# godhj93/bayesian-torch

Measured on AMD Instinct MI355X. Metric: MC-samples/sec (forward+KL), Bayesian-ResNet18 CIFAR batch=128, higher is better.
Workload: dtype f32 (bf16x3 split operands, 6 product terms, f32 accumulate); 1 GPU; cfg3: Bayesian-ResNet18 via dnn_to_bnn (Conv2dReparameterization), CIFAR 3x32x32, batch=128; samples_per_launch=32, batch=128, rng=on-chip philox, parallelism=mc1, output_stage=bn+relu+residual (+ the stem max-pool) folded into the conv kernels, launch=hip graph replay

## Files before the change

### bayesian_torch_amd/_lib.py

```python
import ctypes as C
import os
import threading

import torch

_HERE = os.path.dirname(os.path.abspath(__file__))
LIB_PATH = os.environ.get("BT_LIB_PATH") or os.path.join(_HERE, "libbtorch_hip.so")
WORKSPACE_BYTES = 65536
KL_MAX_SEGMENTS = 64
PACK_MAX_SEGMENTS = 64
KL_RHO_IS_SIGMA = 1
KL_PRIOR_LAPLACE = 2
PRIOR_NORMAL, PRIOR_LAPLACE = 0, 1

_f32p = C.POINTER(C.c_float)
_vp = C.c_void_p


class bt_rng(C.Structure):
    _fields_ = [("seed", C.c_uint64), ("call_base_dev", _vp), ("call", C.c_uint32), ("layer_id", C.c_uint32),
                ("sample0", C.c_uint32), ("reserved", C.c_uint32)]


class bt_params(C.Structure):
# ... 59 lines not shown
    "bt_mc_epilogue": (C.c_int, [C.c_int32, C.c_int32, C.c_int32, _vp, _vp, _vp]),
}
EXPORTS = tuple(_PROTOS)


def lib():
    global _lib
    if _lib is None:
        with _lock:
            if _lib is None:
                if not os.path.exists(LIB_PATH):
                    raise RuntimeError(
                        f"{LIB_PATH} is missing: the HIP extension is the only implementation of this path "
                        "(no CPU/ATen fallback). Build it with `python -c 'import __graft_entry__ as g; g.build()'` "
                        "or `make -C bayesian_torch_amd/csrc`.")
                handle = C.CDLL(LIB_PATH)
                for name, (res, args) in _PROTOS.items():
                    fn = getattr(handle, name)
                    fn.restype, fn.argtypes = res, args
                _lib = handle
    return _lib


LAUNCH_INFO_FIELDS = ("workgroups", "m_tiles", "n_tiles", "S", "t_NI", "t_R", "t_Wt", "pixel_major", "row_tiles", "kl_slices", "groups", "n_bt", "n_rt", "n_ct", "fused_kl")


def last_launch_info():
    v = (C.c_int64 * 16)()
    check(lib().bt_last_launch_info(v, 16))
    return dict(zip(LAUNCH_INFO_FIELDS, (int(x) for x in v)))


ERR_UNSUPPORTED = -2


def check(rc):
    if rc != 0:
        raise RuntimeError(f"libbtorch_hip error {rc}: {lib().bt_last_error_string().decode()}")


def ptr(t):
    return None if t is None else t.data_ptr()


def dev_f32(t, what):
    if t is None:
        return None
# ... 63 lines not shown
```

### bayesian_torch_amd/csrc/bt_fused_api.hip

```cpp
#include <string.h>

#include "bt_fused_fwd.h"

namespace bt {
int launch_reparam(bool linear, const FwdArgs& a, FwdArgs& ran, hipStream_t stream);
int launch_reparam_inj(bool linear, const FwdArgs& a, FwdArgs& ran, hipStream_t stream);
int launch_flipout(bool linear, const FwdArgs& a, FwdArgs& ran, hipStream_t stream);
int launch_flipout_inj(bool linear, const FwdArgs& a, FwdArgs& ran, hipStream_t stream);

static unsigned long long* g_dbg = nullptr;
static thread_local long long g_launch_info[16] = {};
static inline bool al16(const void* p) { return (((uintptr_t)p) & 15u) == 0; }

static int run(bool flip, bool linear, const bt_conv2d_geom& g, int S, const float* x, int64_t x_sample_stride, const bt_params* p,
               const bt_draws* d, const bt_epilogue* ep, float* out, float* kl_out, void* ws, size_t ws_bytes, bt_stream_t stream, const char* who) {
  char msg[256];
  auto bad = [&](const char* what) {
    snprintf(msg, sizeof(msg), "%s: %s", who, what);
    return set_error(BT_ERR_BAD_ARG, msg);
  };
  if (!x || !p || !d || !out) return bad("null argument");
  if (!p->mu_w || !p->rho_w) return bad("mu_w / rho_w are required");
  if ((p->mu_b == nullptr) != (p->rho_b == nullptr)) return bad("mu_b and rho_b must both be given or both be NULL");
  if (S <= 0) return bad("S must be >= 1");
// ... 58 lines not shown
  a.seed_lo = (uint32_t)d->rng.seed, a.seed_hi = (uint32_t)(d->rng.seed >> 32);
  if (ep) a.ep_scale = ep->scale, a.ep_shift = ep->shift, a.ep_res = ep->residual, a.ep_res_stride = ep->residual_sample_stride, a.ep_relu = ep->relu;
  if (ep && ep->pool != BT_POOL_NONE) {
    if (ep->pool != BT_POOL_MAX_3x3_S2_P1) return bad("unknown epilogue pool mode");
    if (linear) return bad("the fused max-pool belongs to the conv2d entry points");
    if (ep->residual) return bad("the fused max-pool takes no residual");
    a.ep_pool = 1, a.ep_Hp = (Ho - 1) / 2 + 1, a.ep_Wp = (Wo - 1) / 2 + 1;
    a.out_elems = (long long)g.B * g.Co * a.ep_Hp * a.ep_Wp;
  }
  a.out_vec4 = (!linear && !a.pixel_major && a.HoWo > 1 && (a.Wo & 3) == 0 && al16(out) && (!a.ep_res || (al16(a.ep_res) && (a.ep_res_stride & 3) == 0)) &&
                (!d->sign_out || al16(d->sign_out))) ? 1 : 0;
  a.dbg = g_dbg;
  a.call = d->rng.call, a.call_base = d->rng.call_base_dev, a.layer_id = d->rng.layer_id, a.sample0 = d->rng.sample0;
  const bool inj = d->eps_w != nullptr;
  const bool all_inj = inj && (!p->mu_b || d->eps_b) && (!flip || (d->sign_in && d->sign_out));
  const bool none_inj = !d->eps_w && !d->eps_b && !d->sign_in && !d->sign_out;
  if (!all_inj && !none_inj) return bad("inject all draws of the layer (eps_w, eps_b when biased, both sign tensors for Flipout) or none");
  if (inj && a.ep_pool) return set_error(BT_ERR_UNSUPPORTED, "fused max-pool: not available with injected draws");
  int rc;
  FwdArgs r;
  if (inj) rc = flip ? launch_flipout_inj(linear, a, r, (hipStream_t)stream) : launch_reparam_inj(linear, a, r, (hipStream_t)stream);
  else rc = flip ? launch_flipout(linear, a, r, (hipStream_t)stream) : launch_reparam(linear, a, r, (hipStream_t)stream);
  if (rc == BT_OK) {
    const long long v[16] = {r.total_blocks, r.m_tiles, r.n_tiles, r.S, r.t_NI, r.t_R, r.t_Wt, r.pixel_major, r.row_taps, r.kl_slices, r.G, r.n_bt, r.n_rt, r.n_ct, r.do_kl, 0};
    for (int i = 0; i < 16; ++i) g_launch_info[i] = v[i];
  }
  if (rc == BT_OK && kl_after) {
    const float* mu[2] = {p->mu_w, p->mu_b};
    const float* rho[2] = {p->rho_w, p->rho_b};
    const float* pm[2] = {p->prior_mu_w, p->prior_mu_b};
    const float* ps[2] = {p->prior_sigma_w, p->prior_sigma_b};
    const int64_t n[2] = {a.w_elems, (int64_t)g.Co};
    const int32_t lay[2] = {0, 0};
    rc = bt_kl_normal(p->mu_b ? 2 : 1, mu, rho, pm, ps, n, lay, BT_KL_PRIOR_LAPLACE, kl_out, ws, ws_bytes, stream);
  }
  return rc;
}

static bt_conv2d_geom linear_geom(int B, int In, int Out) {
  bt_conv2d_geom g;
  g.B = B, g.Ci = In, g.H = 1, g.W = 1, g.Co = Out, g.kh = 1, g.kw = 1;
  g.sh = g.sw = 1, g.ph = g.pw = 0, g.dh = g.dw = 1, g.groups = 1;
  return g;
}
}

extern "C" int bt_reparam_linear_fwd(int32_t B, int32_t In, int32_t Out, int32_t S, const float* x, int64_t x_sample_stride,
// ... 35 lines not shown
```

### bayesian_torch_amd/csrc/bt_fused_fwd.h

```cpp
#pragma once
#include <type_traits>

#include "bt_api_internal.h"

namespace bt {

typedef float f32x16 __attribute__((ext_vector_type(16)));

constexpr int kBK = 36;
constexpr int kMaxTaps = 128;
#ifndef BT_STAMPS
#define BT_STAMPS 0
#endif
constexpr bool kStamps = BT_STAMPS != 0;
constexpr int kThreads = 512;
constexpr int kProducers = 256;

struct FwdArgs {
  const float *x, *mu_w, *rho_w, *mu_b, *rho_b, *pmu_w, *psig_w, *pmu_b, *psig_b;
  const float *mu_pk, *sig_pk;
  const float *eps_w, *eps_b, *sign_in, *sign_out;
  float* out;
  float* kl_out;
  double* slots;
  unsigned* counter;
  long long x_sample_stride, x_elems, out_elems, w_elems;
  int B, Ci, H, W, Co, KH, KW, SH, SW, PH, PW, DH, DW, G;
  int Ho, Wo, HoWo, M, K, Cig, Cog, S, T, HW;
  int n_tiles, m_tiles, total_blocks;
  int t_NI, t_R, t_Wt, n_bt, n_rt, n_ct;
  int patch_ok;
  int x_cvec;
  int x_rows;
  int pixel_major, mt_per_pixel;
  int w_vec, x_vec;
  int do_kl, kl_slices;
  uint32_t seed_lo, seed_hi, call, layer_id, sample0;
  const uint32_t* call_base;
  const float *ep_scale, *ep_shift, *ep_res;
  long long ep_res_stride;
  int ep_relu;
  int ep_pool, ep_Hp, ep_Wp;
  int out_vec4;
  int bn32;
  unsigned long long* dbg;
  uint32_t inv_m_tiles, inv_S, inv_n_tiles, inv_n_bt, inv_n_ct, inv_rw, inv_wt, inv_kw;
  int x_flat;
  int row_taps;
  float* sk_scratch;
  unsigned* sk_tickets;
  long long sk_scratch_bytes;
  int sk_nsl, sk_ks, sk_cpt;
  int sk_kh0, sk_nh, sk_kw0, sk_nw;
  int d_tap;
  int spw, n_sg;
  uint32_t inv_n_sg;
};

inline bool set_grid(FwdArgs& a, long long total) {
  if (total <= 0 || total > 0x7FFFFFFFll) return false;
  a.total_blocks = (int)total;
  a.kl_slices = total < 256 ? (int)total : 256;
  return true;
}

inline bool packed_ok(const FwdArgs& a) {
  return a.mu_pk && !((((uintptr_t)a.mu_pk | (uintptr_t)a.sig_pk) & 15u)) && a.w_elems < (1ll << 29) && a.x_elems < (1ll << 29);
}

__device__ __forceinline__ int xcd_remap(int orig, int n) {
// ... 740 lines not shown
```

### bayesian_torch_amd/csrc/bt_fused_split.h

```cpp
#pragma once
#include "bt_fused_fwd.h"

namespace bt {

typedef short bf16x8 __attribute__((ext_vector_type(8)));

constexpr int kSplitSteps = 5;

template <int BM, bool FLIP = false>
constexpr int split_xpo() {
  return FLIP ? 302 : 1025;
}
template <int BN, int NP, bool FLIP = false>
constexpr int split_w_bytes() { return (FLIP ? 2 : 1) * kSplitSteps * 2 * NP * BN * 16; }
template <int BM, int NP, bool FLIP = false>
constexpr int split_x_bytes() { return split_xpo<BM, FLIP>() * (NP + (FLIP ? 1 : 0)) * 16; }
constexpr int kSplitMiscBytes = kMaxTaps * 16 + 96 + 32 + 64;
template <int BN, int BM, int NP, bool FLIP = false>
constexpr int split_lds_bytes() { return 2 * (split_w_bytes<BN, NP, FLIP>() + split_x_bytes<BM, NP, FLIP>()) + kSplitMiscBytes; }

__device__ __forceinline__ void split_pieces(float v, uint32_t& h, uint32_t& m, uint32_t& l) {
  h = __float_as_uint(v) & 0xFFFF0000u;
  const float r = __fsub_rn(v, __uint_as_float(h));
  m = __float_as_uint(r) & 0xFFFF0000u;
  l = __float_as_uint(__fsub_rn(r, __uint_as_float(m)));
}
__device__ __forceinline__ uint32_t pack_hi16(uint32_t hi, uint32_t lo) {
  return __builtin_amdgcn_perm(hi, lo, 0x07060302u);
}
typedef float f32x2_t __attribute__((ext_vector_type(2)));
typedef uint32_t u32x2_t __attribute__((ext_vector_type(2)));
__device__ __forceinline__ void split_pair(float a, float b, uint32_t& h, uint32_t& m, uint32_t& l) {
  const f32x2_t v = {a, b};
  const u32x2_t hb = __builtin_bit_cast(u32x2_t, v) & 0xFFFF0000u;
  const f32x2_t r = v - __builtin_bit_cast(f32x2_t, hb);
  const u32x2_t mb = __builtin_bit_cast(u32x2_t, r) & 0xFFFF0000u;
  const f32x2_t q = r - __builtin_bit_cast(f32x2_t, mb);
  const u32x2_t lb = __builtin_bit_cast(u32x2_t, q);
  h = pack_hi16(hb.y, hb.x), m = pack_hi16(mb.y, mb.x), l = pack_hi16(lb.y, lb.x);
}

__device__ __forceinline__ int udiv_inv(int n, int d, uint32_t inv) {
  return inv ? (int)__umulhi((uint32_t)n, inv) : (d == 1 ? n : n / d);
}
__device__ __forceinline__ uint32_t inv32(int d) { return 0xFFFFFFFFu / (uint32_t)d + 1u; }
__device__ __forceinline__ int div_small(int n, int d) { return d == 1 ? n : d == 2 ? n >> 1 : n / d; }

template <int BN, int BM, int NP, int NPW, int XM, bool FLIP = false>
__global__ __launch_bounds__(256 + 64 * NPW) void fused_split_kernel(const FwdArgs a) {
  static_assert((BN == 64 && (BM == 512 || BM == 256 || BM == 128)) || (BN == 32 && BM == 128 && !FLIP), "tile shapes of this flavour");
  static_assert(!FLIP || ((BM == 256 || BM == 128) && NP == 3), "Flipout: the 64 x 256 / 64 x 128 tiles, exact split");
  constexpr int kProducers = 64 * NPW, kThreadsAll = 256 + kProducers;
  constexpr int CWM = FLIP ? 2 : 4, CWN = 4 / CWM, WTM = BM / CWM, TN = BN / CWN / 32, TM = WTM / 32;
  constexpr int NOP = FLIP ? 2 : 1;
  constexpr int PB = 16 * (NP + (FLIP ? 1 : 0));
  constexpr int W_BYTES = split_w_bytes<BN, NP, FLIP>(), W_OP = W_BYTES / NOP, X_BYTES = split_x_bytes<BM, NP, FLIP>(), XPO = split_xpo<BM, FLIP>();
  constexpr int W_STEP = 2 * NP * BN * 16, W_HALF = NP * BN * 16, W_PIECE = BN * 16;
  constexpr int SROWS = ((4 * BN + NOP * BN * (BM + 4)) * 4 <= 2 * (W_BYTES + X_BYTES)) ? BN : 32, NPASS = BN / SROWS;
  static_assert(!FLIP || NPASS == 1, "Flipout stages both accumulator sets in one pass");

  extern __shared__ __attribute__((aligned(16))) char smem_c[];
  char* const wbuf = smem_c;
  char* const xbuf = smem_c + 2 * W_BYTES;
  float* const smem = reinterpret_cast<float*>(smem_c);
  int4* const taptab = reinterpret_cast<int4*>(smem_c + 2 * (W_BYTES + X_BYTES));

  unsigned long long* const dbg_ = kStamps ? a.dbg : nullptr;
  const int tid = threadIdx.x, lane = tid & 63, wave = tid >> 6;
  if (dbg_ && dbg_[201] && tid == 0) {
    dbg_[256 + 4 * blockIdx.x] = __builtin_amdgcn_s_memrealtime();
    dbg_[256 + 4 * blockIdx.x + 2] = __builtin_amdgcn_s_memtime();
    dbg_[256 + 4 * blockIdx.x + 3] = (unsigned long long)__builtin_amdgcn_s_getreg((4 << 0) | (0 << 6) | (31 << 11)) |
                                     ((unsigned long long)__builtin_amdgcn_s_getreg((20 << 0) | (0 << 6) | (31 << 11)) << 32);
  }
  const bool stamp0 = dbg_ && blockIdx.x == 0 && (tid == 0 || tid == 256);
  if (stamp0 && tid == 0) dbg_[210] = __builtin_amdgcn_s_memtime();
  const bool producer = wave >= 4;
  const int ptid = producer ? tid - 256 : tid;
  const int li = lane & 31, lh = lane >> 5;
  const int wm = wave & (CWM - 1), wn = (wave & 3) / CWM;

  int L = __builtin_amdgcn_readfirstlane(xcd_remap(blockIdx.x, a.total_blocks));
  int Lq = udiv_inv(L, a.m_tiles, a.inv_m_tiles);
  const int mt = __builtin_amdgcn_readfirstlane(L - Lq * a.m_tiles);
  L = Lq, Lq = udiv_inv(L, a.S, a.inv_S);
  const int s = __builtin_amdgcn_readfirstlane(L - Lq * a.S);
  L = Lq, Lq = udiv_inv(L, a.n_tiles, a.inv_n_tiles);
  const int nt = __builtin_amdgcn_readfirstlane(L - Lq * a.n_tiles);
// ... 65 lines not shown

  const int G8 = Cig >> 3;
  const int ps_h = (dymax == dymin) ? 1 : a.SH, gs_h = (dymax == dymin) ? a.SH : 1;
  const int ps_w = (dxmax == dxmin) ? 1 : a.SW, gs_w = (dxmax == dxmin) ? a.SW : 1;
  const int PHt = (t_R - 1) * ps_h + (dymax - dymin) + 1, PWt = (t_Wt - 1) * ps_w + (dxmax - dxmin) + 1;
  const int x_lo = w0 * a.SW - a.PW + dxmin, y_lo = r0 * a.SH - a.PH + dymin;
  const int kmin_h = y_lo < 0 ? div_small(-y_lo + gs_h - 1, gs_h) : 0, kmin_w = x_lo < 0 ? div_small(-x_lo + gs_w - 1, gs_w) : 0;
  int kmax_h = a.H - 1 - y_lo >= 0 ? div_small(a.H - 1 - y_lo, gs_h) : -1, kmax_w = a.W - 1 - x_lo >= 0 ? div_small(a.W - 1 - x_lo, gs_w) : -1;
  kmax_h = kmax_h < PHt - 1 ? kmax_h : PHt - 1, kmax_w = kmax_w < PWt - 1 ? kmax_w : PWt - 1;
  const int NYR = kmax_h >= kmin_h ? kmax_h - kmin_h + 1 : 0, NXR = kmax_w >= kmin_w ? kmax_w - kmin_w + 1 : 0;
  const int PIMG = NYR * NXR, PCH = t_NI * PIMG;
  constexpr int ZOFF = X_BYTES - PB;
  const int SPO = (nA + 1) >> 1;
  int NO;
  if (nA <= 1) {
    NO = 2 * kSplitSteps;
  } else {
    NO = SPO == 1 ? 5 : SPO == 2 ? 2 : 1;
    static_assert(kSplitSteps == 5, "the table above");
  }
  while (NO > 1 && NO * PCH > XPO - 1) --NO;
  if (nA <= 1 && NO > 1) NO &= ~1;
  if (NO > G8) NO = G8;
  const int NQ = NO * (nA > 0 ? nA : 1);
  const int NSTEP = nA <= 1 ? (NO + 1) >> 1 : NO * SPO;
  const int NS = nA ? (G8 + NO - 1) / NO : 0;
  for (int i = tid; i < 2 * W_BYTES / 16; i += kThreadsAll) reinterpret_cast<uint4*>(smem_c)[i] = make_uint4(0, 0, 0, 0);
  if (tid < 2 * (PB / 16)) reinterpret_cast<uint4*>(xbuf + (tid / (PB / 16)) * X_BYTES + X_BYTES - PB)[tid % (PB / 16)] = make_uint4(0, 0, 0, 0);

  const float* const xs = a.x + (long long)s * a.x_sample_stride;
  constexpr uint32_t kOOB = 0x80000000u;
  auto guard_off = [](bool in, uint32_t off) -> uint32_t {
    const uint32_t m = 0u - (uint32_t)in;
    return (off & m) | (0x80000000u & ~m);
  };
  const int Cig4 = Cig;
  const int pk_bytes = a.Co * T * Cig4 * 4;
  const __amdgpu_buffer_rsrc_t r_mu = __builtin_amdgcn_make_buffer_rsrc(const_cast<float*>(a.mu_pk), 0, pk_bytes, 0x00020000);
  const __amdgpu_buffer_rsrc_t r_rs = __builtin_amdgcn_make_buffer_rsrc(const_cast<float*>(a.sig_pk), 0, pk_bytes, 0x00020000);
  const __amdgpu_buffer_rsrc_t r_x = __builtin_amdgcn_make_buffer_rsrc(const_cast<float*>(xs), 0, (int)(a.x_elems * 4), 0x00020000);
  auto ldf = [](const __amdgpu_buffer_rsrc_t& r, uint32_t byte_off) { return __builtin_bit_cast(float, __builtin_amdgcn_raw_buffer_load_b32(r, (int)byte_off, 0, 0)); };
  auto ldf4 = [](const __amdgpu_buffer_rsrc_t& r, uint32_t byte_off) { return __builtin_bit_cast(float4, __builtin_amdgcn_raw_buffer_load_b128(r, (int)byte_off, 0, 0)); };

  float* const bias0 = smem;
  float* const bias1 = smem + BN;
  float* const osc = smem + 2 * BN;
  float* const osh = smem + 3 * BN;
  const bool kl_block = a.do_kl && (int)blockIdx.x < a.kl_slices;
  float* const out_s = a.out + (long long)s * a.out_elems;
  const float* const res_s = a.ep_res ? a.ep_res + (long long)s * a.ep_res_stride : nullptr;
  const bool relu = a.ep_relu != 0;
// ... 69 lines not shown
      const bool ok = mok && row < rows_ok;
      const uint32_t oi = ok ? obase + (uint32_t)(k * RSTEP * HoWo_) : 0u;
      const int rr = row < SROWS ? k * RSTEP : 0;
      float v = sp[rr * SROW];
      if constexpr (FLIP) {
        const float d = sp[(SROWS + rr) * SROW];
        const int co_l = ok ? co0 + k * RSTEP : 0;
        v = __fadd_rn(__fmul_rn(__fadd_rn(v, __fmul_rn(d, hash_sign(skey_out, oi))), osc[co_l]), osh[co_l]);
      }
      if (res_s && ok) v = __fadd_rn(v, res_s[oi]);
      v = (relu && v < 0.f) ? 0.f : v;
      if (ok) out_s[oi] = v;
    }
  };

  const int prio_mode = dbg_ ? (int)dbg_[200] : 0;
  if (producer) {
    if (prio_mode == 0 && (BM == 512 || FLIP)) __builtin_amdgcn_s_setprio(3);
    constexpr int UMAX = (2 * BN * 2 * kSplitSteps + kProducers - 1) / kProducers;
    const int nunits = 2 * BN * NQ;
    uint32_t e_off[UMAX];
    int l_off[UMAX];
    int u_ol[UMAX];
    bool u_live[UMAX];
    const uint32_t inv_na = nA > 1 ? inv32(nA) : 0u;
#pragma unroll
    for (int i = 0; i < UMAX; ++i) {
      const int u = ptid + kProducers * i;
      const int uu = u < nunits ? u : 0;
      int cq = uu & 1, n = (uu >> 1) & (BN - 1), q = (uu >> 1) / BN;
      if (nA == 1 && NO > 1) {
        const uint32_t inv_no = inv32(NO);
        const int t2 = uu >> 1;
        n = (int)__umulhi((uint32_t)t2, inv_no);
        q = t2 - n * NO;
      }
      const int ol = nA > 1 ? (int)__umulhi((uint32_t)q, inv_na) : q;
      const int ai = nA > 1 ? q - ol * nA : 0;
      const int tap = nA ? taptab[ai].w : 0;
      const int st_ = nA > 1 ? ol * SPO + (ai >> 1) : (ol >> 1), hf = nA > 1 ? (ai & 1) : (ol & 1);
      const int co_g = n0 + n;
      const bool rv = co_g < a.Cog;
      const uint32_t co = (uint32_t)(g * a.Cog + (rv ? co_g : 0));
      e_off[i] = rv ? (co * (uint32_t)T + (uint32_t)tap) * (uint32_t)Cig4 + (uint32_t)(8 * ol + 4 * cq) : (kOOB >> 2);
      l_off[i] = u < nunits ? st_ * W_STEP + hf * W_HALF + (n ^ ((2 * st_ + hf) & 7)) * 16 + cq * 8 : -1;
      u_ol[i] = ol;
      u_live[i] = __builtin_amdgcn_readfirstlane(__ballot(rv && u < nunits) != 0ull ? 1 : 0) != 0;
    }
    const int wave_u0 = __builtin_amdgcn_readfirstlane(ptid & ~63);
    if (stamp0) dbg_[213] = __builtin_amdgcn_s_memtime();
    float4 mu[UMAX], rs[UMAX];
    auto load_w = [&](int st) {
      const int oct0 = st * NO;
#pragma unroll
      for (int i = 0; i < UMAX; ++i) {
        if (u_live[i]) {
          const bool in = l_off[i] >= 0 && oct0 + u_ol[i] < G8 && e_off[i] != (kOOB >> 2);
          const uint32_t sb = guard_off(in, 4u * (e_off[i] + (uint32_t)(8 * oct0)));
          mu[i] = ldf4(r_mu, sb), rs[i] = ldf4(r_rs, sb);
        }
      }
    };
    if (NS > 0) load_w(0);
    constexpr int PIT = (XM == 3 || XM == 4) ? ((XPO - 1) / 2 + kProducers - 1) / kProducers : (XPO - 1 + kProducers - 1) / kProducers;
    constexpr int XV = XM == 3 ? 16 : XM == 4 ? 32 : 8;
    int it_off[PIT], it_lds[PIT], it_ol[PIT];
    const bool flat = XM == 3 && a.x_flat != 0;
    const int ylo_r = y_lo + kmin_h * gs_h, nyr = flat ? 1 : NYR, W4 = flat ? a.HW >> 2 : a.W >> 2;
    const int xpar = (x_lo + kmin_w * gs_w) & 1;
    const int per_oct = XM == 2 ? 4 * t_NI : XM == 3 ? 2 * t_NI * nyr * W4 : XM == 4 ? t_NI * nyr * W4 : PCH;
    const int n_items = NO * per_oct;
    {
      const uint32_t inv_per = per_oct > 1 ? inv32(per_oct) : 0u;
      const uint32_t inv_pimg = PIMG > 0 ? inv32(PIMG) : 0u;
      const uint32_t inv_pw = NXR > 0 ? inv32(NXR) : 0u;
      const int qpi = nyr * W4;
      const uint32_t inv_qpi = qpi > 1 ? inv32(qpi) : 0u;
      const uint32_t inv_w4 = W4 > 1 ? inv32(W4) : 0u;
#pragma unroll
      for (int i = 0; i < PIT; ++i) {
        const int f = ptid + kProducers * i;
        const int ff = f < n_items ? f : 0;
        int ol = per_oct <= 1 ? ff : (int)__umulhi((uint32_t)ff, inv_per);
        int r = ff - ol * per_oct;
        if constexpr (XM == 1) {
          const uint32_t inv_no = NO > 1 ? inv32(NO) : 0u;
          r = NO <= 1 ? ff : (int)__umulhi((uint32_t)ff, inv_no);
          ol = ff - r * NO;
        }
        int pair = 0;
        if constexpr (XM == 2) {
          const int cps = 4 * NO;
          const uint32_t inv_cps = inv32(cps);
          r = (int)__umulhi((uint32_t)ff, inv_cps);
          const int cp = ff - r * cps;
          ol = cp >> 2, pair = cp & 3;
        }
        int off = (int)kOOB, lds = -1;
        if constexpr (XM == 2) {
          const int b = b0 + r;
          lds = (ol * PCH + 4 * r) * PB + 4 * pair;
          if (b < a.B) off = 16 * (b * a.Ci + g * Cig + 2 * pair);
        } else if constexpr (XM == 1) {
          const int b = b0 + r;
          lds = (ol * PCH + r) * PB;
          if (b < a.B) off = 4 * (b * a.Ci + g * Cig);
        } else if constexpr (XM == 3) {
          const int hc = r & 1, q = r >> 1;
          const int img = qpi <= 1 ? q : (int)__umulhi((uint32_t)q, inv_qpi);
          const int rem = q - img * qpi;
          const int yr = W4 <= 1 ? rem : (int)__umulhi((uint32_t)rem, inv_w4);
          const int xq = rem - yr * W4;
          const int b = b0 + img, y = ylo_r + yr * gs_h, x = 4 * xq;
          lds = (ol * PCH + img * PIMG + yr * NXR + x) * PB + hc * 8;
          if (b < a.B) off = 4 * ((b * a.Ci + g * Cig + 4 * hc) * a.HW + y * a.W + x);
        } else if constexpr (XM == 4) {
          const int img = qpi <= 1 ? r : (int)__umulhi((uint32_t)r, inv_qpi);
          const int rem = r - img * qpi;
          const int yr = W4 <= 1 ? rem : (int)__umulhi((uint32_t)rem, inv_w4);
          const int xq = rem - yr * W4;
          const int b = b0 + img, y = ylo_r + yr * gs_h, x = 4 * xq;
          lds = (ol * PCH + img * PIMG + yr * NXR + 2 * xq) * PB;
          if (b < a.B) off = 4 * ((b * a.Ci + g * Cig) * a.HW + y * a.W + x);
        } else {
          const int img = PIMG <= 1 ? r : (int)__umulhi((uint32_t)r, inv_pimg);
          const int rem = r - img * PIMG;
          const int yy = NXR <= 1 ? rem : (int)__umulhi((uint32_t)rem, inv_pw);
          const int xx = rem - yy * NXR;
          const int b = b0 + img, y = y_lo + (yy + kmin_h) * gs_h, x = x_lo + (xx + kmin_w) * gs_w;
          lds = (ol * PCH + r) * PB;
          if (b < a.B) off = 4 * ((b * a.Ci + g * Cig) * a.HW + y * a.W + x);
        }
        it_off[i] = off;
        it_lds[i] = f < n_items ? lds : -1;
        it_ol[i] = ol;
      }
    }
    if (stamp0) dbg_[214] = __builtin_amdgcn_s_memtime();
    const int HWb = 4 * a.HW;
    const int wave_i0 = wave_u0;
    const int n_items_w = n_items;

    float xv[PIT][XV];
    auto load_x = [&](int st) {
      const int oct0 = st * NO;
#pragma unroll
      for (int i = 0; i < PIT; ++i) {
        if (i == 0 || wave_i0 + kProducers * i < n_items_w) {
          const int oc = oct0 + it_ol[i];
          const bool in = it_off[i] != (int)kOOB && oc < G8;
          if constexpr (XM == 2) {
#pragma unroll
            for (int c = 0; c < 2; ++c) {
// ... 77 lines not shown
#pragma unroll
            for (int k = 0; k < 2; ++k) {
              float v[8];
#pragma unroll
              for (int c = 0; c < 8; ++c) v[c] = xpar ? xv[i][4 * c + 2 * k + 1] : xv[i][4 * c + 2 * k];
              store_px(dst + k * PB, v, e0 + (uint32_t)(2 * k + xpar), (uint32_t)a.HW);
            }
          } else {
            const float v[8] = {xv[i][0], xv[i][1], xv[i][2], xv[i][3], xv[i][4], xv[i][5], xv[i][6], xv[i][7]};
            store_px(dst, v, e0, XM == 1 ? 1u : (uint32_t)a.HW);
          }
        }
      }
    };
    if (NS > 0) load_x(0);
    if (stamp0) dbg_[215] = __builtin_amdgcn_s_memtime();
    __syncthreads();
    const bool pstamp = dbg_ && blockIdx.x == 0 && tid == 256;
    for (int st = 0; st <= NS; ++st) {
      if (pstamp && st < 60) dbg_[128 + 2 * st] = __builtin_amdgcn_s_memtime();
      if (pstamp && st == 3) dbg_[250] = dbg_[251] = __builtin_amdgcn_s_memtime();
      if (st < NS) {
        char* const Wt = wbuf + (st & 1) * W_BYTES;
        char* const Xt = xbuf + (st & 1) * X_BYTES;
        const int oct0 = st * NO;
        float ep[UMAX][4];
#pragma unroll
        for (int i = 0; i < UMAX; ++i)
          if (u_live[i])
            philox_normal4(key_w, sample, (e_off[i] + (uint32_t)(8 * oct0)) >> 2, ep[i]);
        if (pstamp && st == 3) dbg_[252] = __builtin_amdgcn_s_memtime();
#pragma unroll
        for (int i = 0; i < UMAX; ++i) {
          if (u_live[i]) {
            const float m4[4] = {mu[i].x, mu[i].y, mu[i].z, mu[i].w}, s4[4] = {rs[i].x, rs[i].y, rs[i].z, rs[i].w};
            uint32_t wh[4], wm_[4], wl[4];
#pragma unroll
            for (int j = 0; j < 4; ++j)
              split_pieces(FLIP ? m4[j] : __fadd_rn(m4[j], __fmul_rn(s4[j], ep[i][j])), wh[j], wm_[j], wl[j]);
            if (l_off[i] >= 0) {
              char* const dst = Wt + l_off[i];
              *reinterpret_cast<uint2*>(dst) = make_uint2(pack_hi16(wh[1], wh[0]), pack_hi16(wh[3], wh[2]));
              *reinterpret_cast<uint2*>(dst + W_PIECE) = make_uint2(pack_hi16(wm_[1], wm_[0]), pack_hi16(wm_[3], wm_[2]));
              if constexpr (NP == 3) *reinterpret_cast<uint2*>(dst + 2 * W_PIECE) = make_uint2(pack_hi16(wl[1], wl[0]), pack_hi16(wl[3], wl[2]));
            }
            if constexpr (FLIP) {
#pragma unroll
              for (int j = 0; j < 4; ++j) split_pieces(__fmul_rn(s4[j], ep[i][j]), wh[j], wm_[j], wl[j]);
              if (l_off[i] >= 0) {
                char* const dst = Wt + W_OP + l_off[i];
                *reinterpret_cast<uint2*>(dst) = make_uint2(pack_hi16(wh[1], wh[0]), pack_hi16(wh[3], wh[2]));
                *reinterpret_cast<uint2*>(dst + W_PIECE) = make_uint2(pack_hi16(wm_[1], wm_[0]), pack_hi16(wm_[3], wm_[2]));
                *reinterpret_cast<uint2*>(dst + 2 * W_PIECE) = make_uint2(pack_hi16(wl[1], wl[0]), pack_hi16(wl[3], wl[2]));
              }
            }
          }
        }
        if (pstamp && st == 3) dbg_[253] = __builtin_amdgcn_s_memtime();
        store_x(Xt, st);
        if (st + 1 < NS) load_x(st + 1), load_w(st + 1);
      }
      if (pstamp && st < 60) dbg_[128 + 2 * st + 1] = __builtin_amdgcn_s_memtime();
      __syncthreads();
    }
    if (ptid < BN) {
      float bv = 0.f;
      const int co_g = n0 + ptid;
      if (a.mu_b && co_g < a.Cog) {
        const int co = g * a.Cog + co_g;
        RngKey kb = key_w;
        kb.layer_tensor = layer_tensor_word(a.layer_id, 1);
        float z[4];
        philox_normal4(kb, sample, (uint32_t)(co >> 2), z);
        const int sel = co & 3;
        const float e = sel == 0 ? z[0] : sel == 1 ? z[1] : sel == 2 ? z[2] : z[3];
        const float dl = __fmul_rn(softplus(a.rho_b[co]), e);
        bv = FLIP ? a.mu_b[co] : __fadd_rn(a.mu_b[co], dl);
        if constexpr (FLIP) bias1[ptid] = dl;
      } else if constexpr (FLIP) {
        bias1[ptid] = 0.f;
      }
      bias0[ptid] = bv;
      const bool cv = a.ep_scale && co_g < a.Cog;
// ... 62 lines not shown
        if (lane == 0) {
          float kl = (float)(t / (double)a.w_elems);
          if (a.mu_b) kl += (float)(bt_ / (double)a.Co);
          a.kl_out[0] = kl;
          __hip_atomic_store(a.counter, 0u, __ATOMIC_RELAXED, __HIP_MEMORY_SCOPE_AGENT);
        }
      }
    };
    int xaddr[TM][kSplitSteps];
    {
      int pimg[TM], pyb[TM], pxb[TM];
      bool live[TM];
#pragma unroll
      for (int j = 0; j < TM; ++j) {
        int b, ho, wo;
        live[j] = col_decode(wm * WTM + j * 32 + li, b, ho, wo);
        pimg[j] = (b - b0) * PIMG, pyb[j] = (ho - r0) * ps_h, pxb[j] = (wo - w0) * ps_w;
      }
#pragma unroll
      for (int q = 0; q < kSplitSteps; ++q) {
        int ol, ai;
        if (nA <= 1) ol = 2 * q + lh, ai = 0;
        else ol = (q >= SPO) + (q >= 2 * SPO) + (q >= 3 * SPO) + (q >= 4 * SPO), ai = 2 * (q - ol * SPO) + lh;
        const bool ent = nA > 0 && ol < NO && ai < nA;
        const int4 e = taptab[ent ? ai : 0];
        const int ty = (dymax == dymin) ? 0 : e.y - dymin, tx = (dxmax == dxmin) ? 0 : e.z - dxmin;
#pragma unroll
        for (int j = 0; j < TM; ++j) {
          const int yy = pyb[j] + ty, xx = pxb[j] + tx;
          const bool ok = ent && live[j] && yy >= kmin_h && yy <= kmax_h && xx >= kmin_w && xx <= kmax_w;
          xaddr[j][q] = ok ? (ol * PCH + pimg[j] + (yy - kmin_h) * NXR + (xx - kmin_w)) * PB : ZOFF;
        }
      }
    }
    int wlq[kSplitSteps];
#pragma unroll
    for (int q = 0; q < kSplitSteps; ++q) wlq[q] = lh * W_HALF + (li ^ ((2 * q + lh) & 7)) * 16 + wn * TN * 32 * 16;

    f32x16 acc[NOP][TN][TM];
#pragma unroll
    for (int o = 0; o < NOP; ++o)
#pragma unroll
      for (int i = 0; i < TN; ++i)
#pragma unroll
        for (int j = 0; j < TM; ++j)
#pragma unroll
          for (int r = 0; r < 16; ++r) acc[o][i][j][r] = 0.f;
    if (prio_mode == 2) __builtin_amdgcn_s_setprio(3);

    const bool cstamp = dbg_ && blockIdx.x == 0 && tid == 0;
    if (cstamp) dbg_[216] = __builtin_amdgcn_s_memtime();
    __syncthreads();
    __syncthreads();
    if (cstamp) dbg_[0] = __builtin_amdgcn_s_memtime();
    for (int st = 0; st < NS; ++st) {
      if (cstamp && st < 60) dbg_[2 + 2 * st] = __builtin_amdgcn_s_memtime();
      const char* const Wt = wbuf + (st & 1) * W_BYTES;
      const char* const Xt = xbuf + (st & 1) * X_BYTES;
      int nstep = NSTEP;
      if ((st + 1) * NO > G8) {
        const int no_l = G8 - st * NO;
        nstep = nA <= 1 ? (no_l + 1) >> 1 : no_l * SPO;
      }
      {
        constexpr int NXP = NP + (FLIP ? 1 : 0);
        bf16x8 wf[2][NOP][TN][NP], xf[2][NXP];
        auto read_w = [&](int q) {
#pragma unroll
          for (int o = 0; o < NOP; ++o)
#pragma unroll
            for (int i = 0; i < TN; ++i)
#pragma unroll
              for (int p = 0; p < NP; ++p)
                wf[q & 1][o][i][p] = *reinterpret_cast<const bf16x8*>(Wt + o * W_OP + wlq[q] + q * W_STEP + p * W_PIECE + i * 32 * 16);
        };
        auto read_x = [&](int u) {
          const char* const px = Xt + xaddr[u % TM][u / TM];
#pragma unroll
          for (int p = 0; p < NXP; ++p) xf[u & 1][p] = *reinterpret_cast<const bf16x8*>(px + 16 * p);
        };
        read_w(0);
        read_x(0);
#pragma unroll
// ... 221 lines not shown
```

### bayesian_torch_amd/csrc/bt_fused_split.hip

```cpp
#include <atomic>
#include <stdlib.h>
#include <string.h>

#include "bt_fused_split_quad.h"
#include "bt_fused_split_direct.h"
#include "bt_fused_split_skinny.h"
#include "bt_fused_split_host.h"

namespace bt {

static std::atomic<int> g_contraction{-1};
int contraction_mode() {
  int m = g_contraction.load(std::memory_order_relaxed);
  if (m < 0) {
    const char* e = getenv("BT_CONTRACTION");
    m = !e ? 0 : (!strcmp(e, "f32") ? 1 : !strcmp(e, "bf16x2") ? 2 : 0);
    g_contraction.store(m, std::memory_order_relaxed);
  }
  return m;
}

template <int BM, int NP, int NPW, int XM, int BN = 64>
static int launch_split_cfg(const FwdArgs& a, hipStream_t stream) {
  constexpr int lds = split_lds_bytes<BN, BM, NP>();
  static_assert(lds <= 160 * 1024, "LDS budget of one CU");
  char nm[160];
  snprintf(nm, sizeof(nm), "fused_split_kernel<%d,%d,bf16x%d,%d terms,npw=%d,xm=%d>", BN, BM, NP, NP == 3 ? 6 : 3, NPW, XM);
  return launch_kernel(fused_split_kernel<BN, BM, NP, NPW, XM>, nm, "fused forward (split)", dim3((unsigned)a.total_blocks), dim3(256 + 64 * NPW),
                       lds, lds, stream, a);
}

template <int BM, int NPW>
static int launch_split_xm(const FwdArgs& a, int mode, int xm, hipStream_t stream) {
  if (mode == 2) return launch_split_cfg<BM, 2, NPW, 0>(a, stream);
  if constexpr (BM == 128) {
    if (a.bn32) {
      if (xm == 1) return launch_split_cfg<BM, 3, NPW, 1, 32>(a, stream);
      if (xm == 2) return launch_split_cfg<BM, 3, NPW, 2, 32>(a, stream);
      return launch_split_cfg<BM, 3, NPW, 0, 32>(a, stream);
    }
    if (xm == 1) return launch_split_cfg<BM, 3, NPW, 1>(a, stream);
    if (xm == 2) return launch_split_cfg<BM, 3, NPW, 2>(a, stream);
  } else {
    if (xm == 3) return launch_split_cfg<BM, 3, NPW, 3>(a, stream);
    if (xm == 4) return launch_split_cfg<BM, 3, NPW, 4>(a, stream);
    if constexpr (BM == 256) {
      if (xm == 2) return launch_split_cfg<BM, 3, 8, 2>(a, stream);
    }
  }
  return launch_split_cfg<BM, 3, NPW, 0>(a, stream);
}

template <bool POOL, bool WALK = false>
static int launch_quad_cfg(const FwdArgs& a, hipStream_t stream) {
  constexpr int lds = split_lds_bytes<64, 512, 3>();
  auto launch = [&](auto kern, const char* nm) {
// ... 129 lines not shown
  ran = a;
  return launch_kernel(fused_split_skinny_kernel,
                       p.ks == 128 ? "fused_split_skinny_kernel<64,4x32,bf16x3,6 terms,split-K 128>" : "fused_split_skinny_kernel<64,4x32,bf16x3,6 terms,split-K 64>",
                       "fused forward (split, skinny)", dim3((unsigned)a.total_blocks), dim3(kSkinnyThreads), skinny_lds_bytes(p.ks), skinny_lds_bytes(128),
                       stream, a);
}

static int launch_split_one(FwdArgs a, FwdArgs& ran, hipStream_t stream) {
  const int mode = contraction_mode();
  if (mode == 1) return 1;
  if (!packed_ok(a)) return 1;
  if (a.Cig <= 4) return launch_quad(a, ran, stream);
  if ((a.Cig & 7) || a.ep_pool) return 1;
  if (mode != 2) {
    const int rck = launch_skinny(a, ran, stream);
    if (rck <= 0) return rck;
    const int rcd = launch_direct(a, ran, stream);
    if (rcd <= 0) return rcd;
  }
  if (a.T > 9) return 1;
  const int Mdom = a.pixel_major ? a.B : a.M;
  if (Mdom < 112) return 1;
  a.n_tiles = (a.Cog + 63) / 64;
  FwdArgs b512 = a, b256 = a, b128 = a;
  const int live512 = Mdom >= 512 ? split_geometry<512>(b512) : 0;
  const int live256 = Mdom >= 256 ? split_geometry<256>(b256) : 0;
  const int live128 = split_geometry<128>(b128);
  const long long per = (long long)a.G * a.n_tiles * a.S;
  const double c512 = split_tile_cost(b512, live512, 512, 256, 96), c256 = split_tile_cost(b256, live256, 256, 256, 96),
               c128 = split_tile_cost(b128, live128, 128, 128, 96);
  int bm = 0;
  static const int force_bm = [] { const char* e = getenv("BT_FORCE_BM"); return e ? atoi(e) : 0; }();
  if (force_bm == 512 && c512 < 1e30) bm = 512;
  else if (force_bm == 256 && c256 < 1e30) bm = 256;
  else if (force_bm == 128 && c128 < 1e30) bm = 128;
  else if (c512 < 1e30 && c512 <= c256 && c512 <= c128) bm = 512;
  else if (c256 < 1e30 && c256 <= c128) bm = 256;
  else if (c128 < 1e30) bm = 128;
  if (!bm) return 1;
  a = bm == 512 ? b512 : bm == 256 ? b256 : b128;
  int bn32_env = g_bn32.load(std::memory_order_relaxed);
  if (bn32_env == -2) {
    const char* e = getenv("BT_BN32");
    bn32_env = e ? (atoi(e) ? 1 : 0) : -1;
    g_bn32.store(bn32_env, std::memory_order_relaxed);
  }
// ... 48 lines not shown
```

### bayesian_torch_amd/csrc/bt_fused_split_host.h

```cpp
#pragma once
#include <stdlib.h>

#include "bt_fused_split.h"

namespace bt {

int contraction_mode();

static inline uint32_t inv_u32(long long d, long long nmax) {
  if (d <= 1 || nmax < 0 || (unsigned long long)nmax * (unsigned long long)d >= (1ull << 32)) return 0u;
  return (uint32_t)(((1ull << 32) + (unsigned long long)d - 1ull) / (unsigned long long)d);
}
static inline void split_fill_inverses(FwdArgs& a) {
  static const bool off = getenv("BT_NO_HOST_INV") != nullptr;
  if (off) {
    a.inv_m_tiles = a.inv_S = a.inv_n_tiles = a.inv_n_bt = a.inv_n_ct = a.inv_rw = a.inv_wt = a.inv_kw = a.inv_n_sg = 0u;
    return;
  }
  const long long tb = a.total_blocks;
  a.inv_m_tiles = inv_u32(a.m_tiles, tb);
  a.inv_S = inv_u32(a.S, tb);
  a.inv_n_tiles = inv_u32(a.n_tiles, tb);
  a.inv_n_bt = inv_u32(a.n_bt, a.m_tiles);
  a.inv_n_ct = inv_u32(a.n_ct, a.m_tiles);
// ... 37 lines not shown
  const int ext = hi - lo, gs = ext ? 1 : S, ps = ext ? S : 1;
  const int x_lo = -P + lo, Pt = (Out - 1) * ps + ext + 1;
  const int kmin = x_lo < 0 ? (-x_lo + gs - 1) / gs : 0;
  int kmax = In - 1 - x_lo >= 0 ? (In - 1 - x_lo) / gs : -1;
  if (kmax > Pt - 1) kmax = Pt - 1;
  *gs_out = gs;
  return kmax >= kmin ? kmax - kmin + 1 : 0;
}
static int split_row_mode(const FwdArgs& a) {
  int gs;
  const int kept = split_axis_kept(a.KW, a.DW, a.SW, a.PW, a.W, a.Wo, &gs);
  if (gs > 2 || (a.W & 3)) return 0;
  if (gs == 1) return kept == a.W ? 3 : 0;
  return kept == a.W / 2 ? 4 : 0;
}
static bool split_rows_cover(const FwdArgs& a) { return split_row_mode(a) == 3; }
static bool split_plane_flat(const FwdArgs& a) {
  if ((a.HW & 3) || a.t_R != a.Ho || a.t_Wt != a.Wo) return false;
  int gh, gw;
  const int kh = split_axis_kept(a.KH, a.DH, a.SH, a.PH, a.H, a.Ho, &gh), kw = split_axis_kept(a.KW, a.DW, a.SW, a.PW, a.W, a.Wo, &gw);
  return gh == 1 && gw == 1 && kh == a.H && kw == a.W;
}

template <int BM, bool FLIP = false>
static int split_geometry(FwdArgs& a) {
  int nh, nw, dys, dxs, nh_min = 0, nw_min = 0;
  tap_window(a.KH, a.DH, a.SH, a.PH, a.H, a.Ho, a.pixel_major != 0 || a.row_taps != 0, &nh, &dys, &nh_min);
  tap_window(a.KW, a.DW, a.SW, a.PW, a.W, a.Wo, a.pixel_major != 0, &nw, &dxs, &nw_min);
  const bool one_tap = a.pixel_major ? nh_min * nw_min <= 1 : nh * nw <= 1;
  const long long XPO = one_tap ? (split_xpo<BM, FLIP>() - 1) / 2 : split_xpo<BM, FLIP>() - 1;
  auto fits = [&](int NI, int R, int Wt) {
    long long PHt = (long long)(R - 1) * (dys ? a.SH : 1) + dys + 1, PWt = (long long)(Wt - 1) * (dxs ? a.SW : 1) + dxs + 1;
    const long long rows_max = dys ? a.H : (a.H - 1) / a.SH + 1, cols_max = dxs ? a.W : (a.W - 1) / a.SW + 1;
    if (PHt > rows_max) PHt = rows_max;
    if (PWt > cols_max) PWt = cols_max;
    return NI * PHt * PWt <= XPO;
  };
  int NI, R, Wt;
  if (a.row_taps) {
    NI = BM / a.Wo, R = 1, Wt = a.Wo;
    if (NI > a.B) NI = a.B;
    if (NI < 1 || !fits(NI, R, Wt)) return 0;
  } else if (a.HoWo == 1 || a.pixel_major) {
    NI = BM, R = 1, Wt = 1;
    if (NI > a.B) NI = a.B;
    if (!fits(NI, R, Wt)) return 0;
  } else if (a.HoWo <= BM) {
    NI = BM / a.HoWo, R = a.Ho, Wt = a.Wo;
    if (NI > a.B) NI = a.B;
    while (NI > 1 && !fits(NI, R, Wt)) --NI;
    if (!fits(NI, R, Wt)) return 0;
  } else if (a.Wo <= BM) {
    NI = 1, R = BM / a.Wo, Wt = a.Wo;
// ... 56 lines not shown
```

Baseline: 18800 MC-samples/s.

## Pair odd tap counts across two channel octets in split conv kernel

Result: faster. 19080 MC-samples/s (median of 6 runs) (+1.5%).

```diff
diff --git a/bayesian_torch_amd/_lib.py b/bayesian_torch_amd/_lib.py
--- a/bayesian_torch_amd/_lib.py
+++ b/bayesian_torch_amd/_lib.py
@@ -105,7 +105,7 @@
     return _lib
 
 
-LAUNCH_INFO_FIELDS = ("workgroups", "m_tiles", "n_tiles", "S", "t_NI", "t_R", "t_Wt", "pixel_major", "row_tiles", "kl_slices", "groups", "n_bt", "n_rt", "n_ct", "fused_kl")
+LAUNCH_INFO_FIELDS = ("workgroups", "m_tiles", "n_tiles", "S", "t_NI", "t_R", "t_Wt", "pixel_major", "row_tiles", "kl_slices", "groups", "n_bt", "n_rt", "n_ct", "fused_kl", "tap_pair")
 
 
 def last_launch_info():
diff --git a/bayesian_torch_amd/csrc/bt_fused_api.hip b/bayesian_torch_amd/csrc/bt_fused_api.hip
--- a/bayesian_torch_amd/csrc/bt_fused_api.hip
+++ b/bayesian_torch_amd/csrc/bt_fused_api.hip
@@ -104,7 +104,7 @@
   if (inj) rc = flip ? launch_flipout_inj(linear, a, r, (hipStream_t)stream) : launch_reparam_inj(linear, a, r, (hipStream_t)stream);
   else rc = flip ? launch_flipout(linear, a, r, (hipStream_t)stream) : launch_reparam(linear, a, r, (hipStream_t)stream);
   if (rc == BT_OK) {
-    const long long v[16] = {r.total_blocks, r.m_tiles, r.n_tiles, r.S, r.t_NI, r.t_R, r.t_Wt, r.pixel_major, r.row_taps, r.kl_slices, r.G, r.n_bt, r.n_rt, r.n_ct, r.do_kl, 0};
+    const long long v[16] = {r.total_blocks, r.m_tiles, r.n_tiles, r.S, r.t_NI, r.t_R, r.t_Wt, r.pixel_major, r.row_taps, r.kl_slices, r.G, r.n_bt, r.n_rt, r.n_ct, r.do_kl, r.tap_pair};
     for (int i = 0; i < 16; ++i) g_launch_info[i] = v[i];
   }
   if (rc == BT_OK && kl_after) {
diff --git a/bayesian_torch_amd/csrc/bt_fused_fwd.h b/bayesian_torch_amd/csrc/bt_fused_fwd.h
--- a/bayesian_torch_amd/csrc/bt_fused_fwd.h
+++ b/bayesian_torch_amd/csrc/bt_fused_fwd.h
@@ -46,6 +46,7 @@
   unsigned long long* dbg;
   uint32_t inv_m_tiles, inv_S, inv_n_tiles, inv_n_bt, inv_n_ct, inv_rw, inv_wt, inv_kw;
   int x_flat;
+  int tap_pair;
   int row_taps;
   float* sk_scratch;
   unsigned* sk_tickets;
diff --git a/bayesian_torch_amd/csrc/bt_fused_split.h b/bayesian_torch_amd/csrc/bt_fused_split.h
--- a/bayesian_torch_amd/csrc/bt_fused_split.h
+++ b/bayesian_torch_amd/csrc/bt_fused_split.h
@@ -15,9 +15,10 @@
 constexpr int split_w_bytes() { return (FLIP ? 2 : 1) * kSplitSteps * 2 * NP * BN * 16; }
 template <int BM, int NP, bool FLIP = false>
 constexpr int split_x_bytes() { return split_xpo<BM, FLIP>() * (NP + (FLIP ? 1 : 0)) * 16; }
+constexpr int kSplitPairPad = 96;
 constexpr int kSplitMiscBytes = kMaxTaps * 16 + 96 + 32 + 64;
 template <int BN, int BM, int NP, bool FLIP = false>
-constexpr int split_lds_bytes() { return 2 * (split_w_bytes<BN, NP, FLIP>() + split_x_bytes<BM, NP, FLIP>()) + kSplitMiscBytes; }
+constexpr int split_lds_bytes() { return 2 * (split_w_bytes<BN, NP, FLIP>() + split_x_bytes<BM, NP, FLIP>()) + (FLIP ? 0 : kSplitPairPad) + kSplitMiscBytes; }
 
 __device__ __forceinline__ void split_pieces(float v, uint32_t& h, uint32_t& m, uint32_t& l) {
   h = __float_as_uint(v) & 0xFFFF0000u;
@@ -46,8 +47,9 @@
 __device__ __forceinline__ uint32_t inv32(int d) { return 0xFFFFFFFFu / (uint32_t)d + 1u; }
 __device__ __forceinline__ int div_small(int n, int d) { return d == 1 ? n : d == 2 ? n >> 1 : n / d; }
 
-template <int BN, int BM, int NP, int NPW, int XM, bool FLIP = false>
+template <int BN, int BM, int NP, int NPW, int XM, bool FLIP = false, bool PAIR = false>
 __global__ __launch_bounds__(256 + 64 * NPW) void fused_split_kernel(const FwdArgs a) {
+  static_assert(!(FLIP && PAIR), "Flipout keeps the unpaired order");
   static_assert((BN == 64 && (BM == 512 || BM == 256 || BM == 128)) || (BN == 32 && BM == 128 && !FLIP), "tile shapes of this flavour");
   static_assert(!FLIP || ((BM == 256 || BM == 128) && NP == 3), "Flipout: the 64 x 256 / 64 x 128 tiles, exact split");
   constexpr int kProducers = 64 * NPW, kThreadsAll = 256 + kProducers;
@@ -63,7 +65,8 @@
   char* const wbuf = smem_c;
   char* const xbuf = smem_c + 2 * W_BYTES;
   float* const smem = reinterpret_cast<float*>(smem_c);
-  int4* const taptab = reinterpret_cast<int4*>(smem_c + 2 * (W_BYTES + X_BYTES));
+  static_assert(FLIP || 2 * PB <= kSplitPairPad, "the paired x buffers' two extra slots fit the pad");
+  int4* const taptab = reinterpret_cast<int4*>(smem_c + 2 * (W_BYTES + X_BYTES) + (FLIP ? 0 : kSplitPairPad));
 
   unsigned long long* const dbg_ = kStamps ? a.dbg : nullptr;
   const int tid = threadIdx.x, lane = tid & 63, wave = tid >> 6;
@@ -175,11 +178,23 @@
   while (NO > 1 && NO * PCH > XPO - 1) --NO;
   if (nA <= 1 && NO > 1) NO &= ~1;
   if (NO > G8) NO = G8;
-  const int NQ = NO * (nA > 0 ? nA : 1);
+  constexpr bool tpair = PAIR;
+  if (PAIR && !(nA > 1 && (nA & 1) && !(G8 & 1) && 2 * PCH <= XPO - 1 && !pix && !a.row_taps)) return;
+  if (tpair) NO = 2;
+  const int PST = tpair ? PCH + 1 : PCH;
+  const int XB_STRIDE = tpair ? X_BYTES + PB : X_BYTES;
+  const int ZTAB = tpair ? PCH * PB : ZOFF;
+  const int NOW = tpair ? 1 : NO;
+  const int NQ = tpair ? nA + 1 : NO * (nA > 0 ? nA : 1);
   const int NSTEP = nA <= 1 ? (NO + 1) >> 1 : NO * SPO;
-  const int NS = nA ? (G8 + NO - 1) / NO : 0;
+  const int NS = !nA ? 0 : tpair ? G8 : (G8 + NO - 1) / NO;
+  const int NXS = tpair ? G8 >> 1 : NS;
   for (int i = tid; i < 2 * W_BYTES / 16; i += kThreadsAll) reinterpret_cast<uint4*>(smem_c)[i] = make_uint4(0, 0, 0, 0);
   if (tid < 2 * (PB / 16)) reinterpret_cast<uint4*>(xbuf + (tid / (PB / 16)) * X_BYTES + X_BYTES - PB)[tid % (PB / 16)] = make_uint4(0, 0, 0, 0);
+  if (tpair && tid < 4 * (PB / 16)) {
+    const int z = tid / (PB / 16);
+    reinterpret_cast<uint4*>(xbuf + (z >> 1) * XB_STRIDE + ((z & 1) * PST + PCH) * PB)[tid % (PB / 16)] = make_uint4(0, 0, 0, 0);
+  }
 
   const float* const xs = a.x + (long long)s * a.x_sample_stride;
   constexpr uint32_t kOOB = 0x80000000u;
@@ -295,6 +310,7 @@
     uint32_t e_off[UMAX];
     int l_off[UMAX];
     int u_ol[UMAX];
+    bool u_liveB[UMAX];
     bool u_live[UMAX];
     const uint32_t inv_na = nA > 1 ? inv32(nA) : 0u;
 #pragma unroll
@@ -308,26 +324,32 @@
         n = (int)__umulhi((uint32_t)t2, inv_no);
         q = t2 - n * NO;
       }
-      const int ol = nA > 1 ? (int)__umulhi((uint32_t)q, inv_na) : q;
-      const int ai = nA > 1 ? q - ol * nA : 0;
+      int ol = nA > 1 ? (int)__umulhi((uint32_t)q, inv_na) : q;
+      int ai = nA > 1 ? q - ol * nA : 0;
+      int st_ = nA > 1 ? ol * SPO + (ai >> 1) : (ol >> 1), hf = nA > 1 ? (ai & 1) : (ol & 1);
+      if (tpair) {
+        ol = q >= nA ? 1 : 0, ai = q >= nA ? nA - 1 : q;
+        st_ = ai >> 1, hf = ol | (ai & 1);
+      }
       const int tap = nA ? taptab[ai].w : 0;
-      const int st_ = nA > 1 ? ol * SPO + (ai >> 1) : (ol >> 1), hf = nA > 1 ? (ai & 1) : (ol & 1);
       const int co_g = n0 + n;
       const bool rv = co_g < a.Cog;
       const uint32_t co = (uint32_t)(g * a.Cog + (rv ? co_g : 0));
       e_off[i] = rv ? (co * (uint32_t)T + (uint32_t)tap) * (uint32_t)Cig4 + (uint32_t)(8 * ol + 4 * cq) : (kOOB >> 2);
       l_off[i] = u < nunits ? st_ * W_STEP + hf * W_HALF + (n ^ ((2 * st_ + hf) & 7)) * 16 + cq * 8 : -1;
       u_ol[i] = ol;
+      u_liveB[i] = __builtin_amdgcn_readfirstlane(__ballot(rv && u < nunits && q < nA - 1) != 0ull ? 1 : 0) != 0;
       u_live[i] = __builtin_amdgcn_readfirstlane(__ballot(rv && u < nunits) != 0ull ? 1 : 0) != 0;
     }
     const int wave_u0 = __builtin_amdgcn_readfirstlane(ptid & ~63);
     if (stamp0) dbg_[213] = __builtin_amdgcn_s_memtime();
     float4 mu[UMAX], rs[UMAX];
     auto load_w = [&](int st) {
-      const int oct0 = st * NO;
+      const int oct0 = st * NOW;
+      const bool stB = tpair && (st & 1);
 #pragma unroll
       for (int i = 0; i < UMAX; ++i) {
-        if (u_live[i]) {
+        if (stB ? u_liveB[i] : u_live[i]) {
           const bool in = l_off[i] >= 0 && oct0 + u_ol[i] < G8 && e_off[i] != (kOOB >> 2);
           const uint32_t sb = guard_off(in, 4u * (e_off[i] + (uint32_t)(8 * oct0)));
           mu[i] = ldf4(r_mu, sb), rs[i] = ldf4(r_rs, sb);
@@ -372,11 +394,11 @@
         int off = (int)kOOB, lds = -1;
         if constexpr (XM == 2) {
           const int b = b0 + r;
-          lds = (ol * PCH + 4 * r) * PB + 4 * pair;
+          lds = (ol * PST + 4 * r) * PB + 4 * pair;
           if (b < a.B) off = 16 * (b * a.Ci + g * Cig + 2 * pair);
         } else if constexpr (XM == 1) {
           const int b = b0 + r;
-          lds = (ol * PCH + r) * PB;
+          lds = (ol * PST + r) * PB;
           if (b < a.B) off = 4 * (b * a.Ci + g * Cig);
         } else if constexpr (XM == 3) {
           const int hc = r & 1, q = r >> 1;
@@ -385,7 +407,7 @@
           const int yr = W4 <= 1 ? rem : (int)__umulhi((uint32_t)rem, inv_w4);
           const int xq = rem - yr * W4;
           const int b = b0 + img, y = ylo_r + yr * gs_h, x = 4 * xq;
-          lds = (ol * PCH + img * PIMG + yr * NXR + x) * PB + hc * 8;
+          lds = (ol * PST + img * PIMG + yr * NXR + x) * PB + hc * 8;
           if (b < a.B) off = 4 * ((b * a.Ci + g * Cig + 4 * hc) * a.HW + y * a.W + x);
         } else if constexpr (XM == 4) {
           const int img = qpi <= 1 ? r : (int)__umulhi((uint32_t)r, inv_qpi);
@@ -393,7 +415,7 @@
           const int yr = W4 <= 1 ? rem : (int)__umulhi((uint32_t)rem, inv_w4);
           const int xq = rem - yr * W4;
           const int b = b0 + img, y = ylo_r + yr * gs_h, x = 4 * xq;
-          lds = (ol * PCH + img * PIMG + yr * NXR + 2 * xq) * PB;
+          lds = (ol * PST + img * PIMG + yr * NXR + 2 * xq) * PB;
           if (b < a.B) off = 4 * ((b * a.Ci + g * Cig) * a.HW + y * a.W + x);
         } else {
           const int img = PIMG <= 1 ? r : (int)__umulhi((uint32_t)r, inv_pimg);
@@ -401,7 +423,7 @@
           const int yy = NXR <= 1 ? rem : (int)__umulhi((uint32_t)rem, inv_pw);
           const int xx = rem - yy * NXR;
           const int b = b0 + img, y = y_lo + (yy + kmin_h) * gs_h, x = x_lo + (xx + kmin_w) * gs_w;
-          lds = (ol * PCH + r) * PB;
+          lds = (ol * PST + r) * PB;
           if (b < a.B) off = 4 * ((b * a.Ci + g * Cig) * a.HW + y * a.W + x);
         }
         it_off[i] = off;
@@ -525,17 +547,17 @@
       if (pstamp && st == 3) dbg_[250] = dbg_[251] = __builtin_amdgcn_s_memtime();
       if (st < NS) {
         char* const Wt = wbuf + (st & 1) * W_BYTES;
-        char* const Xt = xbuf + (st & 1) * X_BYTES;
-        const int oct0 = st * NO;
+        const int oct0 = st * NOW;
+        const bool stB = tpair && (st & 1);
         float ep[UMAX][4];
 #pragma unroll
         for (int i = 0; i < UMAX; ++i)
-          if (u_live[i])
+          if (stB ? u_liveB[i] : u_live[i])
             philox_normal4(key_w, sample, (e_off[i] + (uint32_t)(8 * oct0)) >> 2, ep[i]);
         if (pstamp && st == 3) dbg_[252] = __builtin_amdgcn_s_memtime();
 #pragma unroll
         for (int i = 0; i < UMAX; ++i) {
-          if (u_live[i]) {
+          if (stB ? u_liveB[i] : u_live[i]) {
             const float m4[4] = {mu[i].x, mu[i].y, mu[i].z, mu[i].w}, s4[4] = {rs[i].x, rs[i].y, rs[i].z, rs[i].w};
             uint32_t wh[4], wm_[4], wl[4];
 #pragma unroll
@@ -560,8 +582,15 @@
           }
         }
         if (pstamp && st == 3) dbg_[253] = __builtin_amdgcn_s_memtime();
-        store_x(Xt, st);
-        if (st + 1 < NS) load_x(st + 1), load_w(st + 1);
+        int xs_st = st, xs_ld = st + 1 < NS ? st + 1 : -1;
+        if (tpair) {
+          const int nx = (st + 1) >> 1;
+          xs_st = st == 0 ? 0 : ((st & 1) && nx < NXS ? nx : -1);
+          xs_ld = !(st & 1) && (st >> 1) + 1 < NXS ? (st >> 1) + 1 : -1;
+        }
+        if (xs_st >= 0) store_x(xbuf + (xs_st & 1) * XB_STRIDE, xs_st);
+        if (xs_ld >= 0) load_x(xs_ld);
+        if (st + 1 < NS) load_w(st + 1);
       }
       if (pstamp && st < 60) dbg_[128 + 2 * st + 1] = __builtin_amdgcn_s_memtime();
       __syncthreads();
@@ -670,14 +699,18 @@
         int ol, ai;
         if (nA <= 1) ol = 2 * q + lh, ai = 0;
         else ol = (q >= SPO) + (q >= 2 * SPO) + (q >= 3 * SPO) + (q >= 4 * SPO), ai = 2 * (q - ol * SPO) + lh;
-        const bool ent = nA > 0 && ol < NO && ai < nA;
+        bool ent = nA > 0 && ol < NO && ai < nA;
+        if (tpair) {
+          ent = q < SPO;
+          ol = q == SPO - 1 ? lh : 0, ai = q == SPO - 1 ? nA - 1 : 2 * q + lh;
+        }
         const int4 e = taptab[ent ? ai : 0];
         const int ty = (dymax == dymin) ? 0 : e.y - dymin, tx = (dxmax == dxmin) ? 0 : e.z - dxmin;
 #pragma unroll
         for (int j = 0; j < TM; ++j) {
           const int yy = pyb[j] + ty, xx = pxb[j] + tx;
           const bool ok = ent && live[j] && yy >= kmin_h && yy <= kmax_h && xx >= kmin_w && xx <= kmax_w;
-          xaddr[j][q] = ok ? (ol * PCH + pimg[j] + (yy - kmin_h) * NXR + (xx - kmin_w)) * PB : ZOFF;
+          xaddr[j][q] = ok ? (ol * PST + pimg[j] + (yy - kmin_h) * NXR + (xx - kmin_w)) * PB : ZTAB;
         }
       }
     }
@@ -704,9 +737,11 @@
     for (int st = 0; st < NS; ++st) {
       if (cstamp && st < 60) dbg_[2 + 2 * st] = __builtin_amdgcn_s_memtime();
       const char* const Wt = wbuf + (st & 1) * W_BYTES;
-      const char* const Xt = xbuf + (st & 1) * X_BYTES;
+      const char* const Xt = tpair ? xbuf + ((st >> 1) & 1) * XB_STRIDE + (st & 1) * (PST * PB) : xbuf + (st & 1) * X_BYTES;
       int nstep = NSTEP;
-      if ((st + 1) * NO > G8) {
+      if (tpair) {
+        nstep = SPO - (st & 1);
+      } else if ((st + 1) * NO > G8) {
         const int no_l = G8 - st * NO;
         nstep = nA <= 1 ? (no_l + 1) >> 1 : no_l * SPO;
       }
diff --git a/bayesian_torch_amd/csrc/bt_fused_split.hip b/bayesian_torch_amd/csrc/bt_fused_split.hip
--- a/bayesian_torch_amd/csrc/bt_fused_split.hip
+++ b/bayesian_torch_amd/csrc/bt_fused_split.hip
@@ -20,18 +20,30 @@
   return m;
 }
 
-template <int BM, int NP, int NPW, int XM, int BN = 64>
+template <int BM, int NP, int NPW, int XM, int BN = 64, bool PAIR = false>
 static int launch_split_cfg(const FwdArgs& a, hipStream_t stream) {
   constexpr int lds = split_lds_bytes<BN, BM, NP>();
   static_assert(lds <= 160 * 1024, "LDS budget of one CU");
   char nm[160];
   snprintf(nm, sizeof(nm), "fused_split_kernel<%d,%d,bf16x%d,%d terms,npw=%d,xm=%d>", BN, BM, NP, NP == 3 ? 6 : 3, NPW, XM);
-  return launch_kernel(fused_split_kernel<BN, BM, NP, NPW, XM>, nm, "fused forward (split)", dim3((unsigned)a.total_blocks), dim3(256 + 64 * NPW),
+  return launch_kernel(fused_split_kernel<BN, BM, NP, NPW, XM, false, PAIR>, nm, "fused forward (split)", dim3((unsigned)a.total_blocks), dim3(256 + 64 * NPW),
                        lds, lds, stream, a);
+}
+
+template <int BM, int NPW>
+static int launch_split_pair(const FwdArgs& a, int mode, int xm, hipStream_t stream) {
+  if (mode == 2) return launch_split_cfg<BM, 2, NPW, 0, 64, true>(a, stream);
+  if constexpr (BM == 128) {
+    if (a.bn32) return launch_split_cfg<BM, 3, NPW, 0, 32, true>(a, stream);
+  } else {
+    if (xm == 3) return launch_split_cfg<BM, 3, NPW, 3, 64, true>(a, stream);
+  }
+  return launch_split_cfg<BM, 3, NPW, 0, 64, true>(a, stream);
 }
 
 template <int BM, int NPW>
 static int launch_split_xm(const FwdArgs& a, int mode, int xm, hipStream_t stream) {
+  if (a.tap_pair) return launch_split_pair<BM, NPW>(a, mode, xm, stream);
   if (mode == 2) return launch_split_cfg<BM, 2, NPW, 0>(a, stream);
   if constexpr (BM == 128) {
     if (a.bn32) {
@@ -207,6 +219,7 @@
   const int Mdom = a.pixel_major ? a.B : a.M;
   if (Mdom < 112) return 1;
   a.n_tiles = (a.Cog + 63) / 64;
+  a.tap_pair = split_tap_pair(a) ? 1 : 0;
   FwdArgs b512 = a, b256 = a, b128 = a;
   const int live512 = Mdom >= 512 ? split_geometry<512>(b512) : 0;
   const int live256 = Mdom >= 256 ? split_geometry<256>(b256) : 0;
diff --git a/bayesian_torch_amd/csrc/bt_fused_split_host.h b/bayesian_torch_amd/csrc/bt_fused_split_host.h
--- a/bayesian_torch_amd/csrc/bt_fused_split_host.h
+++ b/bayesian_torch_amd/csrc/bt_fused_split_host.h
@@ -83,13 +83,25 @@
   return gh == 1 && gw == 1 && kh == a.H && kw == a.W;
 }
 
+static bool split_tap_pair(const FwdArgs& a) {
+  static const bool off = [] { const char* e = getenv("BT_NO_TAP_PAIR"); return e && *e && *e != '0'; }();
+  if (off || a.pixel_major || a.row_taps || a.ep_pool) return false;
+  if (a.SH != 1 || a.SW != 1 || a.DH != 1 || a.DW != 1 || a.H > a.Ho || a.W > a.Wo || a.HoWo > 128 || a.HoWo <= 4) return false;
+  if ((a.Cig & 15) || a.T > 9) return false;
+  int nh, nw, eh, ew;
+  tap_window(a.KH, a.DH, a.SH, a.PH, a.H, a.Ho, false, &nh, &eh);
+  tap_window(a.KW, a.DW, a.SW, a.PW, a.W, a.Wo, false, &nw, &ew);
+  const int nA = nh * nw;
+  return nA > 1 && (nA & 1);
+}
+
 template <int BM, bool FLIP = false>
 static int split_geometry(FwdArgs& a) {
   int nh, nw, dys, dxs, nh_min = 0, nw_min = 0;
   tap_window(a.KH, a.DH, a.SH, a.PH, a.H, a.Ho, a.pixel_major != 0 || a.row_taps != 0, &nh, &dys, &nh_min);
   tap_window(a.KW, a.DW, a.SW, a.PW, a.W, a.Wo, a.pixel_major != 0, &nw, &dxs, &nw_min);
   const bool one_tap = a.pixel_major ? nh_min * nw_min <= 1 : nh * nw <= 1;
-  const long long XPO = one_tap ? (split_xpo<BM, FLIP>() - 1) / 2 : split_xpo<BM, FLIP>() - 1;
+  const long long XPO = (one_tap || (!FLIP && a.tap_pair)) ? (split_xpo<BM, FLIP>() - 1) / 2 : split_xpo<BM, FLIP>() - 1;
   auto fits = [&](int NI, int R, int Wt) {
     long long PHt = (long long)(R - 1) * (dys ? a.SH : 1) + dys + 1, PWt = (long long)(Wt - 1) * (dxs ? a.SW : 1) + dxs + 1;
     const long long rows_max = dys ? a.H : (a.H - 1) / a.SH + 1, cols_max = dxs ? a.W : (a.W - 1) / a.SW + 1;
```
